# WangFeng18/3d-gaussian-splatting

Measured on NVIDIA H100. Metric: render+backward FPS @1080p (2.4M Gaussians), higher is better.
Workload: dtype f32

## Files before the change

### 3d-gaussian-splatting_b200/csrc/blend.cu

```cuda
#include <cstdlib>
#include <type_traits>

#include "internal.h"

namespace {

constexpr int FWD_THREADS = 64;
constexpr int FWD_PX = 4;
constexpr int FWD_STAGES = 2;

template <int FWD_CH>
struct FwdSmem {
  float4 A[FWD_STAGES][FWD_CH];
  float4 C[FWD_STAGES][FWD_CH];
  float2 B[FWD_STAGES][FWD_CH + 2];
  uint64_t full[FWD_STAGES];
};

template <typename SM, int CH>
__device__ __forceinline__ void issue_chunk(SM& sm, int stage, const float4* __restrict__ pA,
                                            const float2* __restrict__ pB, const float4* __restrict__ pC,
                                            int base, int n, int shift) {
  uint32_t bytes_a = (uint32_t)n * 16u;
  uint32_t nb = (uint32_t)(n + shift + 1) & ~1u;
// ... 26 lines not shown
    return make_float2(t.x, t.y);
  }
  __device__ __forceinline__ float4 c(int j) const {
    const float4 t = R[j * recw + 1];
    return make_float4(t.z, t.w, R[j * recw + 2].x, 0.f);
  }
  __device__ __forceinline__ float depth(int j) const { return R[j * recw + 2].y; }
  __device__ __forceinline__ uint32_t slot(int j, int tx, int ty) const {
    const float4 cc = R[j * recw + 2];
    const uint32_t rxy = __float_as_uint(cc.z), rwh = __float_as_uint(cc.w);
    const uint32_t off = __float_as_uint(R[j * recw + 3].x);
    return off + ((uint32_t)ty - (rxy >> 16)) * (rwh & 0xffffu) + ((uint32_t)tx - (rxy & 0xffffu));
  }
};

template <int CH, int STAGES, int RECW>
struct GatherRing {
  float4 rec[STAGES][CH * RECW];
  uint64_t full[STAGES];
};

template <int NT, int CH>
struct GatherIds {
  uint32_t id[(CH + NT - 1) / NT];
  __device__ __forceinline__ void load(const uint32_t* __restrict__ ids, int base, int n, int tid) {
#pragma unroll
    for (int u = 0; u < (CH + NT - 1) / NT; ++u) {
      const int i = tid + u * NT;
      id[u] = i < n ? __ldg(ids + base + i) : 0u;
    }
  }
};

template <typename SM, int NT, int CH, int RECW>
__device__ __forceinline__ void gather_issue(SM& sm, int stage, const GsRec* __restrict__ grec,
                                             const uint32_t* __restrict__ goff, const GatherIds<NT, CH>& g, int n,
                                             int tid) {
#pragma unroll
  for (int u = 0; u < (CH + NT - 1) / NT; ++u) {
    const int i = tid + u * NT;
    if (i < n) {
      const float4* src = reinterpret_cast<const float4*>(grec + g.id[u]);
      const uint32_t dst = gs_smem_u32(&sm.rec[stage][i * RECW]);
#pragma unroll
      for (int q = 0; q < 3; ++q)
        asm volatile("cp.async.cg.shared.global [%0], [%1], 16;" ::"r"(dst + 16u * q), "l"(src + q) : "memory");
      if (RECW == 4)
        asm volatile("cp.async.ca.shared.global [%0], [%1], 4;" ::"r"(dst + 48u), "l"(goff + g.id[u]) : "memory");
    }
  }
  asm volatile("cp.async.mbarrier.arrive.noinc.shared::cta.b64 [%0];" ::"r"(gs_smem_u32(&sm.full[stage])) : "memory");
}

template <int FWD_CH, int PX, bool GATHER, bool AUX = false, bool BATCH = false>
__device__ __forceinline__ void blend_fwd_body(const float4* __restrict__ pA, const float2* __restrict__ pB,
                                               const float4* __restrict__ pC, const GsRec* __restrict__ grec,
                                               const uint32_t* __restrict__ ids, const int* __restrict__ tile_accum,
                                               int wp, int hp, int ntx, float fx, float fy, float* __restrict__ image,
                                               int* __restrict__ tile_neff, float* __restrict__ final_img, GsCrop crop,
                                               GsAuxOut aux, const GsView* __restrict__ views) {
  static_assert(!AUX || GATHER, "the aux outputs read |p_c| from the gathered records");
  static_assert(!BATCH || GATHER, "batched frames run the gather path");
  using Smem = typename std::conditional<GATHER, GatherRing<FWD_CH, FWD_STAGES, 3>, FwdSmem<FWD_CH>>::type;
  __shared__ __align__(16) Smem sm;
  const int tile = blockIdx.x;
  const int tid = threadIdx.x;
  const int tx = tile % ntx, ty = tile / ntx;
  int lty = ty;
  if constexpr (BATCH) {
    const int v = ty / (hp / GS_TILE);
    lty = ty - v * (hp / GS_TILE);
    fx = views[v].fx;
    fy = views[v].fy;
    if (final_img) final_img += (size_t)v * crop.width * crop.height * 3;
    if (aux.aux_final) aux.aux_final += (size_t)v * crop.width * crop.height * 2;
  }
  constexpr int FWD_PX = PX, TPR = GS_TILE / PX, NTHREADS = 256 / PX;
  const int ix0 = tx * GS_TILE + (tid % TPR) * FWD_PX;
  const int iy = ty * GS_TILE + (tid / TPR);
  const int iyv = lty * GS_TILE + (tid / TPR);
  float px[FWD_PX];
#pragma unroll
  for (int p = 0; p < FWD_PX; ++p) px[p] = gs_pixel_coord(ix0 + p, wp, fx);
  const float py = gs_pixel_coord(iyv, hp, fy);

  const int start = tile_accum[tile];
  const int cnt = tile_accum[tile + 1] - start;
  const int shift = start & 1;
  const int nchunks = (cnt + FWD_CH - 1) / FWD_CH;

  if (tid == 0) {
    for (int s = 0; s < FWD_STAGES; ++s) gs_mbar_init(&sm.full[s], GATHER ? NTHREADS : 1);
    gs_fence_barrier_init();
  }
  __syncthreads();
  GatherIds<NTHREADS, FWD_CH> gid;
  if constexpr (GATHER) {
    for (int k = 0; k < FWD_STAGES && k < nchunks; ++k) {
      gid.load(ids, start + k * FWD_CH, min(FWD_CH, cnt - k * FWD_CH), tid);
      gather_issue<Smem, NTHREADS, FWD_CH, 3>(sm, k, grec, nullptr, gid, min(FWD_CH, cnt - k * FWD_CH), tid);
    }
    if (FWD_STAGES < nchunks) gid.load(ids, start + FWD_STAGES * FWD_CH, min(FWD_CH, cnt - FWD_STAGES * FWD_CH), tid);
  } else if (tid == 0) {
    for (int k = 0; k < FWD_STAGES && k < nchunks; ++k)
      issue_chunk<Smem, FWD_CH>(sm, k, pA, pB, pC, start + k * FWD_CH, min(FWD_CH, cnt - k * FWD_CH), shift);
  }

  float T[FWD_PX], cr[FWD_PX], cg[FWD_PX], cb[FWD_PX], dep[FWD_PX];
#pragma unroll
  for (int p = 0; p < FWD_PX; ++p) {
    T[p] = 1.f;
    cr[p] = cg[p] = cb[p] = 0.f;
    dep[p] = 0.f;
  }
  int consumed = cnt;
  int k = 0;
  for (; k < nchunks; ++k) {
    const int stage = k % FWD_STAGES;
    gs_mbar_wait(&sm.full[stage], (uint32_t)((k / FWD_STAGES) & 1));
    const int n = min(FWD_CH, cnt - k * FWD_CH);
    StageView<GATHER> sv;
    if constexpr (GATHER) {
      sv.R = sm.rec[stage];
      sv.recw = 3;
    } else {
      sv.A = sm.A[stage];
      sv.C = sm.C[stage];
      sv.B = sm.B[stage] + shift;
    }

#define GS_FWD_BODY(J)                                                                      \
  {                                                                                         \
    const float4 a = sv.a(J);                                                               \
    const float2 b = sv.b(J);                                                               \
    const float4 c = sv.c(J);                                                               \
    const float dy = py - a.y;                                                              \
    const float m1 = a.w * dy;                                                              \
    const float ev = fmaf(-b.x * dy, dy, b.y);                                              \
    float t = 0.f;                                                                          \
    if constexpr (AUX) t = sv.depth(J);                                                     \
    _Pragma("unroll") for (int p = 0; p < FWD_PX; ++p) {                                    \
      const float dx = px[p] - a.x;                                                         \
      const float eu = fmaf(a.z, dx, -m1);                                                  \
      const float alpha = gs_ex2(fmaf(-dx, eu, ev));  \
      const float w = (T[p] > GS_T_STOP) ? alpha * T[p] : 0.f;                              \
      cr[p] = fmaf(c.x, w, cr[p]);                                                          \
      cg[p] = fmaf(c.y, w, cg[p]);                                                          \
      cb[p] = fmaf(c.z, w, cb[p]);                                                          \
      if constexpr (AUX) dep[p] = fmaf(t, w, dep[p]);                                       \
      T[p] -= w;                                                                            \
    }                                                                                       \
  }
    int j = 0;
    bool warp_dead = false;
    for (; j + 4 <= n; j += 4) {
#pragma unroll
      for (int u = 0; u < 4; ++u) GS_FWD_BODY(j + u)
      bool dead = true;
#pragma unroll
      for (int p = 0; p < FWD_PX; ++p) dead = dead && !(T[p] > GS_T_STOP);
      if (__all_sync(0xffffffffu, dead)) {
        warp_dead = true;
        break;
      }
    }
    if (!warp_dead)
      for (; j < n; ++j) GS_FWD_BODY(j)
#undef GS_FWD_BODY

    bool dead = true;
#pragma unroll
    for (int p = 0; p < FWD_PX; ++p) dead = dead && !(T[p] > GS_T_STOP);
    const int all_dead = NTHREADS == 32 ? __all_sync(0xffffffffu, dead) : __syncthreads_and(dead);
    if (NTHREADS == 32) __syncwarp();
    if (all_dead) {
      consumed = min(cnt, (k + 1) * FWD_CH);
      break;
    }
    if (k + FWD_STAGES < nchunks) {
      const int kn = k + FWD_STAGES;
      if constexpr (GATHER) {
        gather_issue<Smem, NTHREADS, FWD_CH, 3>(sm, stage, grec, nullptr, gid, min(FWD_CH, cnt - kn * FWD_CH), tid);
        if (kn + 1 < nchunks) gid.load(ids, start + (kn + 1) * FWD_CH, min(FWD_CH, cnt - (kn + 1) * FWD_CH), tid);
      } else if (tid == 0)
        issue_chunk<Smem, FWD_CH>(sm, stage, pA, pB, pC, start + kn * FWD_CH, min(FWD_CH, cnt - kn * FWD_CH), shift);
    }
  }
  if (tid == 0 && k < nchunks) {
    for (int kk = k + 1; kk < nchunks && kk < k + FWD_STAGES; ++kk)
      gs_mbar_wait(&sm.full[kk % FWD_STAGES], (uint32_t)((kk / FWD_STAGES) & 1));
  }
  if constexpr (AUX) {
#pragma unroll
    for (int p = 0; p < FWD_PX; ++p) {
      cr[p] = fmaf(T[p], aux.bg[0], cr[p]);
      cg[p] = fmaf(T[p], aux.bg[1], cg[p]);
      cb[p] = fmaf(T[p], aux.bg[2], cb[p]);
    }
    float ab[FWD_PX * 2];
#pragma unroll
    for (int p = 0; p < FWD_PX; ++p) {
      ab[2 * p] = dep[p];
      ab[2 * p + 1] = 1.f - T[p];
    }
    if (aux.aux) {
      float4* o = reinterpret_cast<float4*>(aux.aux + ((size_t)iy * wp + ix0) * 2);
#pragma unroll
      for (int q = 0; q < FWD_PX / 2; ++q) o[q] = make_float4(ab[4 * q], ab[4 * q + 1], ab[4 * q + 2], ab[4 * q + 3]);
    }
    if (aux.aux_final) {
#pragma unroll
      for (int p = 0; p < FWD_PX; ++p) {
        const int x = ix0 + p - crop.left, y = iyv - crop.top;
        if (x >= 0 && x < crop.width && y >= 0 && y < crop.height)
          *reinterpret_cast<float2*>(aux.aux_final + ((size_t)y * crop.width + x) * 2) = make_float2(ab[2 * p], ab[2 * p + 1]);
      }
    }
  }
  {
    float ob[FWD_PX * 3];
#pragma unroll
    for (int p = 0; p < FWD_PX; ++p) {
      ob[3 * p] = cr[p];
      ob[3 * p + 1] = cg[p];
      ob[3 * p + 2] = cb[p];
    }
    float4* o = reinterpret_cast<float4*>(image + ((size_t)iy * wp + ix0) * 3);
#pragma unroll
    for (int q = 0; q < FWD_PX * 3 / 4; ++q) o[q] = make_float4(ob[4 * q], ob[4 * q + 1], ob[4 * q + 2], ob[4 * q + 3]);
  }
  if (final_img) {
#pragma unroll
    for (int p = 0; p < FWD_PX; ++p)
      gs_store_final(final_img, ix0 + p, iyv, crop.left, crop.top, crop.width, crop.height, cr[p], cg[p], cb[p]);
  }
  if (tile_neff && tid == 0) tile_neff[tile] = consumed;
}

template <int FWD_CH, int PX, bool GATHER, bool AUX = false>
__global__ void __launch_bounds__(256 / PX) blend_fwd_kernel(const float4* __restrict__ pA,
                                                                 const float2* __restrict__ pB,
                                                                 const float4* __restrict__ pC,
                                                                 const GsRec* __restrict__ grec,
                                                                 const uint32_t* __restrict__ ids,
                                                                 const int* __restrict__ tile_accum, int wp, int hp,
                                                                 int ntx, float fx, float fy,
                                                                 float* __restrict__ image,
                                                                 int* __restrict__ tile_neff,
                                                                 float* __restrict__ final_img, GsCrop crop,
                                                                 GsAuxOut aux) {
  blend_fwd_body<FWD_CH, PX, GATHER, AUX>(pA, pB, pC, grec, ids, tile_accum, wp, hp, ntx, fx, fy, image, tile_neff,
                                          final_img, crop, aux, nullptr);
}

template <bool AUX>
__global__ void __launch_bounds__(64) blend_fwd_batch_kernel(const GsRec* __restrict__ grec,
                                                             const uint32_t* __restrict__ ids,
                                                             const int* __restrict__ tile_accum, int wp, int hp,
                                                             int ntx, const GsView* __restrict__ views,
                                                             float* __restrict__ image, int* __restrict__ tile_neff,
                                                             float* __restrict__ final_img, GsCrop crop, GsAuxOut aux) {
  blend_fwd_body<128, 4, true, AUX, true>(nullptr, nullptr, nullptr, grec, ids, tile_accum, wp, hp, ntx, 0.f, 0.f,
                                          image, tile_neff, final_img, crop, aux, views);
}

constexpr int BWD_STAGES = 2;
constexpr int BWD_NV = 9;

template <int WARPS, int BWD_CH>
struct BwdSmem {
  float4 A[BWD_STAGES][BWD_CH];
  float4 C[BWD_STAGES][BWD_CH];
  float2 B[BWD_STAGES][BWD_CH + 2];
  uint64_t full[BWD_STAGES];
  float partial[WARPS][BWD_CH * BWD_NV];
};

template <int WARPS, int BWD_CH>
__global__ void __launch_bounds__(32 * WARPS) blend_bwd_kernel(const float4* __restrict__ pA,
                                                                const float2* __restrict__ pB,
                                                                const float4* __restrict__ pC,
                                                                const int* __restrict__ tile_accum, int wp, int hp,
                                                                int ntx, float fx, float fy,
                                                                const float* __restrict__ image,
                                                                const float* __restrict__ grad_image,
                                                                float* __restrict__ grad_inst, int grad_is_final,
                                                                GsCrop crop, uint32_t* __restrict__ row_epoch,
                                                                uint32_t epoch, int* __restrict__ tile_neff_b) {
  constexpr int THREADS = 32 * WARPS;
  constexpr int PX = 256 / THREADS;
  constexpr int TPR = GS_TILE / PX;
  using Smem = BwdSmem<WARPS, BWD_CH>;
  __shared__ __align__(16) Smem sm;
  const int tile = blockIdx.x;
  const int tid = threadIdx.x, warp = tid >> 5, lane = tid & 31;
  const int tx = tile % ntx, ty = tile / ntx;
  const int start = tile_accum[tile];
  const int cnt = tile_accum[tile + 1] - start;
  if (cnt == 0) return;
  const int shift = start & 1;
  const int nchunks = (cnt + BWD_CH - 1) / BWD_CH;

  const int ix0 = tx * GS_TILE + (tid % TPR) * PX;
  const int iy = ty * GS_TILE + (tid / TPR);
  float px[PX];
#pragma unroll
  for (int p = 0; p < PX; ++p) px[p] = gs_pixel_coord(ix0 + p, wp, fx);
  const float py = gs_pixel_coord(iy, hp, fy);

  float T[PX], R[PX], gr[PX], gg[PX], gb[PX];
  {
    const size_t off = ((size_t)iy * wp + ix0) * 3;
    const float4* im = reinterpret_cast<const float4*>(image + off);
    float gbuf[PX * 3], ibuf[PX * 3];
#pragma unroll
    for (int q = 0; q < PX * 3 / 4; ++q) {
// ... 958 lines not shown
                                                                      float* __restrict__ g_cov) {
  int i = blockIdx.x * 256 + threadIdx.x;
  if (i >= m) return;
  const float* row = grad_inst + (size_t)i * gw;
  float4 cv = reinterpret_cast<const float4*>(cov)[i];
  float det = cv.x * cv.w - cv.y * cv.z;
  double pn = 2.0 * (double)det + 1e-14;
  float sc = (float)((double)GS_LOG2E / pn);
  float kk = 2.f * sc * sc / GS_LOG2E;
  float d_ca = row[2], d_cb = row[3], d_cc = row[4];
  float gsc = d_ca * cv.w + d_cb * (cv.y + cv.z) + d_cc * cv.x;
  g_pos[3 * i] = row[0];
  g_pos[3 * i + 1] = row[1];
  reinterpret_cast<float4*>(g_cov)[i] = make_float4(d_cc * sc - gsc * kk * cv.w, d_cb * sc + gsc * kk * cv.z,
                                                    d_cb * sc + gsc * kk * cv.y, d_ca * sc - gsc * kk * cv.x);
  g_opa[i] = opa[i] > 0.f ? row[5] / (opa[i] * GS_LN2) : 0.f;
  for (int q = 0; q < d; ++q) g_rgb[(size_t)i * d + q] = row[6 + q];
}

struct LegacyWs {
  float4* pA;
  float2* pB;
  float4* pC;
  float* grad_inst;
};

inline size_t align_up(size_t x, size_t a) { return (x + a - 1) / a * a; }

inline size_t legacy_ws_layout(int m, int d, LegacyWs* ws, char* base) {
  size_t off = 0;
  size_t mm = (size_t)(m > 0 ? m : 0);
  size_t crow = d == 3 ? 16 : (size_t)gs_sh_stream_width(d) * 4;
  size_t grow = d == 3 ? (size_t)GS_GREC * 4 : (size_t)gs_sh_grad_width(d) * 4;
  if (ws) ws->pA = reinterpret_cast<float4*>(base + off);
  off += align_up(mm * 16, 256);
  if (ws) ws->pC = reinterpret_cast<float4*>(base + off);
  off += align_up(mm * crow + 16, 256);
  if (ws) ws->pB = reinterpret_cast<float2*>(base + off);
  off += align_up((mm + 2) * 8, 256);
  if (ws) ws->grad_inst = reinterpret_cast<float*>(base + off);
  off += align_up(mm * grow, 256);
  return off;
}

}

cudaError_t gs_launch_blend_fwd(const float4* pA, const float2* pB, const float4* pC, const GsRec* grec,
                                const uint32_t* ids, const int* tile_accum, const GsFrameGeom& g, float* image,
                                int* tile_neff, float* final_img, const GsCrop& crop, cudaStream_t st,
                                const GsAuxOut* aux) {
  const GsTuning& tn = gs_tuning();
  const bool gather = grec != nullptr;
  if (aux) {
    blend_fwd_kernel<128, 4, true, true><<<g.n_tiles, 64, 0, st>>>(pA, pB, pC, grec, ids, tile_accum, g.wp, g.hp, g.ntx,
                                                                  g.fx, g.fy, image, tile_neff, final_img, crop, *aux);
    return cudaGetLastError();
  }
  if (!gather && tn.fwd_kernel != 0) {
    blend_fwd_ws_kernel<<<g.n_tiles, WSF_CONS + 32, 0, st>>>(pA, pB, pC, tile_accum, g.wp, g.hp, g.ntx, g.fx, g.fy, image,
                                                             tile_neff, final_img, crop);
    return cudaGetLastError();
  }
  const int ch = tn.fwd_ch;
#define GS_FWD_LAUNCH(CH, PX, GA)                                                                                   \
  blend_fwd_kernel<CH, PX, GA><<<g.n_tiles, 256 / PX, 0, st>>>(pA, pB, pC, grec, ids, tile_accum, g.wp, g.hp, g.ntx, \
                                                               g.fx, g.fy, image, tile_neff, final_img, crop, GsAuxOut{})
#define GS_FWD_CH(PX, GA)                     \
  if (ch == 64) GS_FWD_LAUNCH(64, PX, GA);    \
  else if (ch == 256) GS_FWD_LAUNCH(256, PX, GA); \
  else GS_FWD_LAUNCH(128, PX, GA)
  if (gather) {
    if (tn.fwd_px == 8) { GS_FWD_CH(8, true); } else { GS_FWD_CH(4, true); }
  } else {
    if (tn.fwd_px == 8) { GS_FWD_CH(8, false); } else { GS_FWD_CH(4, false); }
  }
#undef GS_FWD_CH
#undef GS_FWD_LAUNCH
  return cudaGetLastError();
}

cudaError_t gs_launch_blend_bwd(const float4* pA, const float2* pB, const float4* pC, const GsRec* grec,
                                const uint32_t* ids, const uint32_t* goff, const int* tile_accum, const GsFrameGeom& g,
                                const float* image,
                                const float* grad_image, float* grad_inst, int grad_is_final, const GsCrop& crop,
                                uint32_t* row_epoch, uint32_t epoch, int* tile_neff_b, cudaStream_t st,
                                const float* aux, const float* grad_aux, bool absgrad) {
  const GsTuning& tn = gs_tuning();
  const bool gather = grec != nullptr;
  if (gather && !row_epoch) return cudaErrorInvalidValue;
  if (absgrad) {
    if (!gather || (grad_aux && !aux)) return cudaErrorInvalidValue;
#define GS_BWD2_ABS(AX, RP)                                                                                        \
  blend_bwd2_kernel<8, false, 4, 3, 10, 4, true, 32, AX, RP, true><<<g.n_tiles, 32, 0, st>>>(                       \
      pA, pB, pC, grec, ids, goff, tile_accum, g.wp, g.hp, g.ntx, g.fx, g.fy, image, grad_image, grad_inst,         \
      grad_is_final, crop, row_epoch, epoch, tile_neff_b, aux, grad_aux)
    if (grad_aux && tn.blend_repack) GS_BWD2_ABS(true, true);
    else if (grad_aux) GS_BWD2_ABS(true, false);
    else if (tn.blend_repack) GS_BWD2_ABS(false, true);
    else GS_BWD2_ABS(false, false);
#undef GS_BWD2_ABS
    return cudaGetLastError();
  }
  if (grad_aux) {
    if (!gather || !aux) return cudaErrorInvalidValue;
#define GS_BWD2_AUX(RP)                                                                                            \
  blend_bwd2_kernel<8, false, 4, 3, 10, 4, true, 32, true, RP><<<g.n_tiles, 32, 0, st>>>(                           \
      pA, pB, pC, grec, ids, goff, tile_accum, g.wp, g.hp, g.ntx, g.fx, g.fy, image, grad_image, grad_inst,         \
      grad_is_final, crop, row_epoch, epoch, tile_neff_b, aux, grad_aux)
    if (tn.blend_repack) GS_BWD2_AUX(true);
    else GS_BWD2_AUX(false);
#undef GS_BWD2_AUX
    return cudaGetLastError();
  }
  if (tn.bwd_kernel != 0 || gather) {
#define GS_BWD2C(PX, WS, UNR, ST, MINB, RQ, GA, CH)                                                                 \
  blend_bwd2_kernel<PX, WS, UNR, ST, MINB, RQ, GA, CH><<<g.n_tiles, 256 / PX + (WS ? 32 : 0), 0, st>>>(              \
      pA, pB, pC, grec, ids, goff, tile_accum, g.wp, g.hp, g.ntx, g.fx, g.fy, image, grad_image, grad_inst,          \
      grad_is_final,                                                                                                 \
      crop, row_epoch, epoch, tile_neff_b, nullptr, nullptr)
#define GS_BWD2(PX, WS, UNR, ST, MINB, RQ, GA) GS_BWD2C(PX, WS, UNR, ST, MINB, RQ, GA, 64)
    const int key = ((((tn.bwd_px * 10 + tn.bwd_ws) * 10 + tn.bwd_unroll) * 10 + tn.bwd_stages) * 10 + tn.bwd_rq) * 100 +
                    tn.bwd_minb;
    if (gather && tn.bwd_ch == 32) {
#define GS_BWD2_SHIPPED()                                                                                          \
  if (tn.blend_repack)                                                                                             \
// ... 72 lines not shown

static bool shipped_rgb_bwd_knobs(const GsTuning& tn) {
  return tn.bwd_kernel != 0 && tn.bwd_px == 8 && tn.bwd_ws == 0 && tn.bwd_unroll == 4 && tn.bwd_stages == 3 &&
         tn.bwd_rq == 4 && tn.bwd_minb == 10 && tn.bwd_ch == 32;
}

int gs_blend_aux_supported(int d, bool forward, bool backward) {
  const GsTuning& tn = gs_tuning();
  if (!tn.gather)
    return gs_set_error_msg(GS_ERR_UNSUPPORTED, "depth / alpha / background: the packed path (gs_tune(\"gather\", 0)) has no aux kernel");
  if (d != 3) {
    if (backward && (gs_sh_tc_mode(d) & 6) == 6)
      return gs_set_error_msg(GS_ERR_UNSUPPORTED,
                              "depth / alpha gradients: the two-pixel tensor-core SH backward (sh_tc bit 2) has no aux kernel");
    return 0;
  }
  if (forward && (tn.fwd_kernel != 0 || tn.fwd_ch != 128 || tn.fwd_px != 4))
    return gs_set_error_msg(GS_ERR_UNSUPPORTED,
                            "depth / alpha / background: only the shipped forward blend knobs (fwd_kernel 0, fwd_ch 128, fwd_px 4) have an aux kernel");
  if (backward && !shipped_rgb_bwd_knobs(tn))
    return gs_set_error_msg(GS_ERR_UNSUPPORTED,
                            "depth / alpha gradients: only the shipped backward blend knobs have an aux kernel");
  return 0;
}

int gs_blend_absgrad_supported(int d, bool gather) {
  const GsTuning& tn = gs_tuning();
  if (d != 3)
    return gs_set_error_msg(GS_ERR_UNSUPPORTED,
                            "densify statistics: absgrad needs the RGB blend (RGB or per-Gaussian SH colour); SH colour "
                            "evaluated per pixel has only grad2d");
  if (!gather)
    return gs_set_error_msg(GS_ERR_UNSUPPORTED,
                            "densify statistics: absgrad is not available on the packed path (gs_tune(\"gather\", 0))");
  if (!shipped_rgb_bwd_knobs(tn))
    return gs_set_error_msg(GS_ERR_UNSUPPORTED,
                            "densify statistics: absgrad needs the shipped backward blend knobs");
  return 0;
}

int gs_blend_batch_supported() {
  const GsTuning& tn = gs_tuning();
  if (!tn.gather)
    return gs_set_error_msg(GS_ERR_UNSUPPORTED, "batched frame: the packed path (gs_tune(\"gather\", 0)) has no batched kernel");
  if (tn.fwd_kernel != 0 || tn.fwd_ch != 128 || tn.fwd_px != 4 || !shipped_rgb_bwd_knobs(tn) || !tn.blend_repack)
    return gs_set_error_msg(GS_ERR_UNSUPPORTED,
                            "batched frame: only the shipped RGB blend knobs (with the live-pixel repack) have batched kernels");
  return 0;
}

cudaError_t gs_launch_blend_fwd_batch(const GsRec* grec, const uint32_t* ids, const int* tile_accum,
                                      const GsFrameGeom& g, const GsView* views, float* image, int* tile_neff,
                                      float* final_img, const GsCrop& crop, cudaStream_t st, const GsAuxOut* aux) {
  if (aux)
    blend_fwd_batch_kernel<true><<<g.n_tiles, 64, 0, st>>>(grec, ids, tile_accum, g.wp, g.hp, g.ntx, views, image,
                                                           tile_neff, final_img, crop, *aux);
  else
    blend_fwd_batch_kernel<false><<<g.n_tiles, 64, 0, st>>>(grec, ids, tile_accum, g.wp, g.hp, g.ntx, views, image,
                                                            tile_neff, final_img, crop, GsAuxOut{});
  return cudaGetLastError();
}

cudaError_t gs_launch_blend_bwd_batch(const GsRec* grec, const uint32_t* ids, const uint32_t* goff,
                                      const int* tile_accum, const GsFrameGeom& g, const GsView* views,
                                      const float* image, const float* grad_image, float* grad_inst, int grad_is_final,
                                      const GsCrop& crop, uint32_t* row_epoch, uint32_t epoch, int* tile_neff_b,
                                      cudaStream_t st, const float* aux, const float* grad_aux, bool absgrad) {
  if (!row_epoch || (grad_aux && !aux)) return cudaErrorInvalidValue;
#define GS_BWD2_BATCH(AX, AB)                                                                                      \
  blend_bwd2_batch_kernel<AX, AB><<<g.n_tiles, 32, 0, st>>>(nullptr, nullptr, nullptr, grec, ids, goff, tile_accum, \
                                                            g.wp, g.hp, g.ntx, 0.f, 0.f, image, grad_image,         \
                                                            grad_inst, grad_is_final, crop, row_epoch, epoch,       \
                                                            tile_neff_b, aux, grad_aux, views)
  if (grad_aux && absgrad) GS_BWD2_BATCH(true, true);
  else if (grad_aux) GS_BWD2_BATCH(true, false);
  else if (absgrad) GS_BWD2_BATCH(false, true);
  else GS_BWD2_BATCH(false, false);
#undef GS_BWD2_BATCH
  return cudaGetLastError();
}

extern "C" size_t gs_draw_workspace_bytes(int m, int d) {
  if (d != 3 && gs_sh_basis_count(d) == 0) return 0;
  return legacy_ws_layout(m, d, nullptr, nullptr);
}

static int check_draw_args(const char* fn, int m, int d, int wp, int hp, int weight_normalize, int sigmoid,
                           size_t ws_bytes, void* ws) {
  if (m < 0 || wp <= 0 || hp <= 0 || (wp % GS_TILE) || (hp % GS_TILE))
    return gs_set_error_msg(GS_ERR_INVALID_ARG, fn);
  if (weight_normalize || sigmoid || (d != 3 && gs_sh_basis_count(d) == 0)) return gs_set_error_msg(GS_ERR_UNSUPPORTED, fn);
  if (m > 0 && (ws == nullptr || ws_bytes < gs_draw_workspace_bytes(m, d)))
    return gs_set_error_msg(GS_ERR_INVALID_ARG, fn);
  return 0;
}

extern "C" int gs_draw_fwd(const float* pos, const float* rgb, const float* opa, const float* cov,
                           const int* tile_n_point_accum, int m, int d, int width_padded, int height_padded,
                           float focal_x, float focal_y, int weight_normalize, int sigmoid, const float* rays_o,
                           const float* lefttop, const float* vec_dx, const float* vec_dy, float* image,
                           void* workspace, size_t workspace_bytes, gs_stream_t stream) {
  int rc = check_draw_args("gs_draw_fwd: bad/unsupported arguments", m, d, width_padded, height_padded,
                           weight_normalize, sigmoid, workspace_bytes, workspace);
  if (rc) return rc;
  if (d != 3 && (!rays_o || !lefttop || !vec_dx || !vec_dy))
    return gs_set_error_msg(GS_ERR_INVALID_ARG, "gs_draw_fwd: SH colour needs rays_o / lefttop / vec_dx / vec_dy");
  cudaStream_t st = (cudaStream_t)stream;
  LegacyWs ws{};
  legacy_ws_layout(m, d, &ws, static_cast<char*>(workspace));
  if (m > 0) {
    if (d == 3)
      legacy_pack_kernel<<<(m + 255) / 256, 256, 0, st>>>(pos, rgb, opa, cov, m, ws.pA, ws.pB, ws.pC);
// ... 77 lines not shown
```

### 3d-gaussian-splatting_b200/csrc/internal.h

```cpp
#pragma once
#include <cuda_runtime.h>
#include <stdint.h>

#include "../../include/gs_b200.h"
#include "project.cuh"

#define GS_GREC 12

struct GsFrameGeom {
  int width, height, wp, hp, ntx, nty, n_tiles;
  float fx, fy;
};

struct GsCrop {
  int left, top, width, height;
};

struct GsAuxOut {
  float bg[3];
  float* aux;
  float* aux_final;
};

#ifdef __CUDACC__
__device__ __forceinline__ void gs_store_aux(const GsAuxOut& ax, int ix, int iy, int wp, const GsCrop& crop,
                                             float depth, float alpha) {
  if (ax.aux) *reinterpret_cast<float2*>(ax.aux + ((size_t)iy * wp + ix) * 2) = make_float2(depth, alpha);
  const int x = ix - crop.left, y = iy - crop.top;
  if (ax.aux_final && x >= 0 && x < crop.width && y >= 0 && y < crop.height)
    *reinterpret_cast<float2*>(ax.aux_final + ((size_t)y * crop.width + x) * 2) = make_float2(depth, alpha);
}
template <int PX>
__device__ __forceinline__ void gs_load_aux_grad(const float* __restrict__ aux, const float* __restrict__ grad_aux,
                                                 int grad_is_final, int ix0, int iy, int wp, const GsCrop& crop,
                                                 float (&gD)[PX], float (&gA)[PX], float (&R)[PX]) {
#pragma unroll
  for (int p = 0; p < PX; ++p) {
    const size_t off = ((size_t)iy * wp + ix0 + p) * 2;
    const float2 da = *reinterpret_cast<const float2*>(aux + off);
    float2 g = make_float2(0.f, 0.f);
    if (!grad_is_final) {
      g = *reinterpret_cast<const float2*>(grad_aux + off);
    } else {
      const int x = ix0 + p - crop.left, y = iy - crop.top;
      if (x >= 0 && x < crop.width && y >= 0 && y < crop.height)
        g = *reinterpret_cast<const float2*>(grad_aux + ((size_t)y * crop.width + x) * 2);
    }
    gD[p] = g.x;
    gA[p] = g.y;
    R[p] = fmaf(g.x, da.x, fmaf(g.y, da.y, R[p]));
  }
}
#endif

struct GsRayPtrs {
  const float *rays_o, *lefttop, *dx, *dy;
};

struct GsTuning {
  int fwd_kernel;
  int fwd_ch;
  int bwd_kernel;
  int bwd_px;
  int bwd_ws;
  int bwd_unroll;
  int bwd_stages;
  int bwd_minb;
  int bwd_rq;
  int fwd_px;
  int bwd_ch;
  int strict;
  int gather;
  int sh_tc;
  int blend_repack;
};
GsTuning& gs_tuning();

void gs_count_launch(int n = 1);

int gs_sh_basis_count(int d);
int gs_sh_stream_width(int d);
int gs_sh_grad_width(int d);
int gs_sh_tc_mode(int d);
cudaError_t gs_launch_blend_sh_fwd(const float4* pA, const float2* pB, const float* pS, const GsRec* grec,
                                   const float* rgb, const uint32_t* ids, const uint32_t* goff , int d,
                                   const int* tile_accum,
                                   const GsFrameGeom& g, const GsRayPtrs& r, float* image, int* tile_neff,
                                   float* final_img, const GsCrop& crop, cudaStream_t st,
                                   const GsAuxOut* aux = nullptr );
cudaError_t gs_launch_blend_sh_bwd(const float4* pA, const float2* pB, const float* pS, const GsRec* grec,
                                   const float* rgb, const uint32_t* ids, const uint32_t* goff , int d,
                                   const int* tile_accum,
                                   const GsFrameGeom& g, const GsRayPtrs& r, const float* image,
                                   const float* grad_image, float* grad_inst, int grad_is_final, const GsCrop& crop,
                                   uint32_t* row_epoch, uint32_t epoch, int* tile_neff_b, cudaStream_t st,
                                   const float* aux = nullptr, const float* grad_aux = nullptr );

cudaError_t gs_launch_blend_sh_fwd_tc(const GsRec* grec, const float* rgb, const uint32_t* ids, int d,
                                      const int* tile_accum, const GsFrameGeom& g, const GsRayPtrs& r, float* image,
                                      int* tile_neff, float* final_img, const GsCrop& crop, cudaStream_t st,
                                      const GsAuxOut* aux = nullptr);
cudaError_t gs_launch_blend_sh_bwd_tc(const GsRec* grec, const float* rgb, const uint32_t* ids, const uint32_t* goff, int d,
                                      const int* tile_accum, const GsFrameGeom& g, const GsRayPtrs& r, const float* image,
                                      const float* grad_image, float* grad_inst, int grad_is_final, const GsCrop& crop,
                                      uint32_t* row_epoch, uint32_t epoch, int* tile_neff_b, cudaStream_t st,
                                      const float* aux = nullptr, const float* grad_aux = nullptr);

cudaError_t gs_launch_fused_project(const float* pos, const float* rgb, const float* opa, const float* quat,
                                    const float* scale, int n, int d, int scale_act, const GsCam& cam,
                                    const GsTileGrid& grid, float near_plane, float half_w, float half_h,
                                    GsRec* rec, uint2* rect ,
                                    uint32_t* count, uint32_t* dkey, int64_t* mask, unsigned int* n_visible, cudaStream_t st,
                                    bool sh_gaussian = false ,
                                    const GsFilter2d* filt = nullptr );

struct GsView {
  GsCam cam;
  GsTileGrid grid;
  GsFilter2d filt;
  float half_w, half_h, fx, fy;
};

cudaError_t gs_launch_fused_project_batch(const float* pos, const float* rgb, const float* opa, const float* quat,
                                          const float* scale, int n, int n_views, int d, int scale_act,
                                          const GsView* views, float near_plane, GsRec* rec ,
                                          uint2* rect , uint32_t* count , uint32_t* dkey ,
                                          int64_t* mask , unsigned int* n_visible,
// ... 116 lines not shown
```

### 3d-gaussian-splatting_b200/csrc/render.cu

```cuda
#include <cub/device/device_radix_sort.cuh>
#include <cub/device/device_scan.cuh>
#include <cub/iterator/counting_input_iterator.cuh>
#include <cub/iterator/transform_input_iterator.cuh>

#include <cmath>
#include <cstdio>
#include <cstdlib>
#include <cstring>
#include <new>

#include "internal.h"

struct GsCountInSortedOrder {
  const uint32_t* count;
  const uint32_t* perm;
  uint32_t n;
  __host__ __device__ __forceinline__ uint32_t operator()(uint32_t i) const { return i < n ? count[perm[i]] : 0u; }
};

static thread_local char g_err[512] = {0};

int gs_set_error(cudaError_t e, const char* what) {
  snprintf(g_err, sizeof(g_err), "CUDA error %d (%s) at %s", (int)e, cudaGetErrorString(e), what);
  return (int)e;
}
int gs_set_error_msg(int code, const char* what) {
  snprintf(g_err, sizeof(g_err), "%s", what);
  return code;
}
extern "C" const char* gs_last_error(void) { return g_err; }
extern "C" int gs_abi_version(void) { return 2; }

static int tune_env(const char* name, int dflt) {
  const char* e = getenv(name);
  return e ? atoi(e) : dflt;
}
GsTuning& gs_tuning() {
  static GsTuning t = {tune_env("GS_TUNE_FWD_KERNEL", 0),  tune_env("GS_TUNE_FWD_CH", 128),   tune_env("GS_TUNE_BWD_KERNEL", 1),
                       tune_env("GS_TUNE_BWD_PX", 8),      tune_env("GS_TUNE_BWD_WS", 0),     tune_env("GS_TUNE_BWD_UNROLL", 4),
                       tune_env("GS_TUNE_BWD_STAGES", 3),  tune_env("GS_TUNE_BWD_MINB", 10),  tune_env("GS_TUNE_BWD_RQ", 4),
                       tune_env("GS_TUNE_FWD_PX", 4),      tune_env("GS_TUNE_BWD_CH", 32),    tune_env("GS_TUNE_STRICT", 0),
                       tune_env("GS_TUNE_GATHER", 1),      tune_env("GS_TUNE_SH_TC", -1),     tune_env("GS_TUNE_BLEND_REPACK", 1)};
  return t;
}
extern "C" int gs_tune(const char* name, int value) {
  if (!name) return gs_set_error_msg(GS_ERR_INVALID_ARG, "gs_tune: null name");
  GsTuning& t = gs_tuning();
  struct { const char* k; int* v; } tab[] = {{"fwd_kernel", &t.fwd_kernel}, {"fwd_ch", &t.fwd_ch},
                                             {"bwd_kernel", &t.bwd_kernel}, {"bwd_px", &t.bwd_px},
                                             {"bwd_ws", &t.bwd_ws},         {"bwd_unroll", &t.bwd_unroll},
                                             {"bwd_stages", &t.bwd_stages}, {"bwd_minb", &t.bwd_minb},
                                             {"bwd_rq", &t.bwd_rq},         {"fwd_px", &t.fwd_px},
                                             {"gather", &t.gather},         {"bwd_ch", &t.bwd_ch},
                                             {"strict", &t.strict},         {"sh_tc", &t.sh_tc},
                                             {"blend_repack", &t.blend_repack}};
  for (auto& e : tab)
    if (!strcmp(e.k, name)) {
      *e.v = value;
      return 0;
    }
  return gs_set_error_msg(GS_ERR_INVALID_ARG, "gs_tune: unknown knob");
}

#include <atomic>
static std::atomic<unsigned long long> g_launches{0};
void gs_count_launch(int n) { g_launches.fetch_add((unsigned long long)n, std::memory_order_relaxed); }
extern "C" unsigned long long gs_kernel_launches(void) { return g_launches.load(std::memory_order_relaxed); }

struct GsAllocator {
  gs_alloc_fn alloc = nullptr;
  gs_free_fn free = nullptr;
  void* user = nullptr;
};
static thread_local const GsAllocator* g_cur_alloc = nullptr;

struct DevBuf {
  void* p = nullptr;
  size_t cap = 0;
  const GsAllocator* owner = nullptr;
  void drop(cudaStream_t st, bool sync) {
    if (!p) return;
    if (owner && owner->free) {
      owner->free(p, owner->user);
    } else {
      if (sync) cudaStreamSynchronize(st);
      cudaFree(p);
    }
    p = nullptr;
    cap = 0;
  }
  cudaError_t reserve(size_t bytes, cudaStream_t st) {
    if (bytes <= cap) return cudaSuccess;
    drop(st, true);
    size_t want = bytes + bytes / 8 + 256;
    const GsAllocator* a = g_cur_alloc;
    if (a && a->alloc) {
      p = a->alloc(want, a->user, (gs_stream_t)st);
      if (!p) return cudaErrorMemoryAllocation;
      owner = a;
    } else {
      cudaError_t e = cudaMalloc(&p, want);
      if (e != cudaSuccess) return e;
      owner = nullptr;
    }
    cap = want;
    return cudaSuccess;
  }
  void release() { drop(nullptr, false); }
// ... 1004 lines not shown
```

Measured before the change: 488.7.

## Repack live pixels across warp lanes in forward blend as pixels saturate

Adds a forward-blend repacking step. At segment and chunk boundaries, each warp counts the pixels that are still unsaturated. When enough have terminated, it retires the finished pixels by writing them to the image, then redistributes the survivors so each lane holds 2 or 1 pixels via warp shuffles. This targets wasted alpha-blend work on lanes whose pixels have already hit the transmittance cutoff. The cost is shuffle-heavy bookkeeping, more code paths specialised on pixel count, and scattered pixel stores. It is enabled by default through a new tuning knob.

```diff
diff --git a/3d-gaussian-splatting_b200/csrc/blend.cu b/3d-gaussian-splatting_b200/csrc/blend.cu
--- a/3d-gaussian-splatting_b200/csrc/blend.cu
+++ b/3d-gaussian-splatting_b200/csrc/blend.cu
@@ -102,7 +102,113 @@
   asm volatile("cp.async.mbarrier.arrive.noinc.shared::cta.b64 [%0];" ::"r"(gs_smem_u32(&sm.full[stage])) : "memory");
 }
 
-template <int FWD_CH, int PX, bool GATHER, bool AUX = false, bool BATCH = false>
+constexpr int FWD_RP = 32;
+
+template <bool AUX, typename Retire>
+__device__ __forceinline__ void fwd_repack(int warp, int lane, int& S, int& row, uint32_t& cols, int& npx,
+                                           float (&px)[4], float& py, float (&T)[4], float (&cr)[4], float (&cg)[4],
+                                           float (&cb)[4], float (&dep)[4], Retire&& retire) {
+  uint32_t mask = 0;
+#pragma unroll
+  for (int p = 0; p < 4; ++p) mask |= T[p] > GS_T_STOP ? 1u << p : 0u;
+  const int c = __popc(mask);
+  if (__reduce_add_sync(0xffffffffu, c) > 16 * S) return;
+  const int wr = row - 8 * warp;
+  int live = 0;
+#pragma unroll
+  for (int r = 0; r < 8; ++r) {
+    const int v = __reduce_add_sync(0xffffffffu, wr == r ? c : 0);
+    if (lane == r) live = v;
+  }
+  int ns = S;
+  while (ns > 1 && __reduce_add_sync(0xffffffffu, (live + ns / 2 - 1) / (ns / 2)) <= 32) ns /= 2;
+  if (ns == S) return;
+
+#pragma unroll
+  for (int p = 0; p < 4; ++p)
+    if (p < npx && !((mask >> p) & 1u)) retire((int)((cols >> (4 * p)) & 15u), row, T[p], cr[p], cg[p], cb[p], dep[p]);
+  int excl = c;
+#pragma unroll
+  for (int o = 1; o < 32; o <<= 1) {
+    const int t = __shfl_up_sync(0xffffffffu, excl, o);
+    if (lane >= o) excl += t;
+  }
+  excl -= c;
+  int sc = (((live + ns - 1) / ns) << 16) | live;
+  const int own = sc;
+#pragma unroll
+  for (int o = 1; o < 8; o <<= 1) {
+    const int t = __shfl_up_sync(0xffffffffu, sc, o);
+    if (lane >= o) sc += t;
+  }
+  sc -= own;
+  int nr = GS_TILE, src = 0, n = 0;
+#pragma unroll
+  for (int r = 0; r < 8; ++r) {
+    const int s = __shfl_sync(0xffffffffu, sc, r), lr = __shfl_sync(0xffffffffu, live, r);
+    const int q = lane - (s >> 16);
+    if (q >= 0 && q * ns < lr) {
+      nr = 8 * warp + r;
+      src = (s & 0xffff) + q * ns;
+      n = min(ns, lr - q * ns);
+    }
+  }
+  int sl[2], sp[2];
+  uint32_t ncols = 0;
+#pragma unroll
+  for (int q = 0; q < 2; ++q) {
+    const int e = src + q;
+    int l = 0;
+#pragma unroll
+    for (int b = 16; b > 0; b >>= 1) {
+      const int t = __shfl_sync(0xffffffffu, excl, (l + b) & 31);
+      if (l + b < 32 && t <= e) l += b;
+    }
+    const int k = e - __shfl_sync(0xffffffffu, excl, l);
+    const uint32_t m = __shfl_sync(0xffffffffu, mask, l);
+    const uint32_t cl = __shfl_sync(0xffffffffu, cols, l);
+    int pos = 0, cnt = 0;
+#pragma unroll
+    for (int p = 0; p < 4; ++p)
+      if ((m >> p) & 1u) {
+        if (cnt == k) pos = p;
+        ++cnt;
+      }
+    sl[q] = l;
+    sp[q] = pos;
+    if (q < n) ncols |= ((cl >> (4 * pos)) & 15u) << (4 * q);
+  }
+  const float npy = __shfl_sync(0xffffffffu, py, sl[0]);
+  auto move = [&](float (&v)[4]) {
+    float nv[2];
+#pragma unroll
+    for (int q = 0; q < 2; ++q) {
+      float acc = 0.f;
+#pragma unroll
+      for (int p = 0; p < 4; ++p) {
+        const float t = __shfl_sync(0xffffffffu, v[p], sl[q]);
+        if (sp[q] == p) acc = t;
+      }
+      nv[q] = q < n ? acc : 0.f;
+    }
+    v[0] = nv[0];
+    v[1] = nv[1];
+    v[2] = v[3] = 0.f;
+  };
+  move(px);
+  move(T);
+  move(cr);
+  move(cg);
+  move(cb);
+  if constexpr (AUX) move(dep);
+  if (n) py = npy;
+  row = nr;
+  cols = ncols;
+  npx = n;
+  S = ns;
+}
+
+template <int FWD_CH, int PX, bool GATHER, bool AUX = false, bool BATCH = false, bool REPACK = false>
 __device__ __forceinline__ void blend_fwd_body(const float4* __restrict__ pA, const float2* __restrict__ pB,
                                                const float4* __restrict__ pC, const GsRec* __restrict__ grec,
                                                const uint32_t* __restrict__ ids, const int* __restrict__ tile_accum,
@@ -111,6 +217,7 @@
                                                GsAuxOut aux, const GsView* __restrict__ views) {
   static_assert(!AUX || GATHER, "the aux outputs read |p_c| from the gathered records");
   static_assert(!BATCH || GATHER, "batched frames run the gather path");
+  static_assert(!REPACK || (GATHER && PX == 4 && FWD_CH % FWD_RP == 0), "the repack deals 4-pixel lanes at segment ends");
   using Smem = typename std::conditional<GATHER, GatherRing<FWD_CH, FWD_STAGES, 3>, FwdSmem<FWD_CH>>::type;
   __shared__ __align__(16) Smem sm;
   const int tile = blockIdx.x;
@@ -132,7 +239,10 @@
   float px[FWD_PX];
 #pragma unroll
   for (int p = 0; p < FWD_PX; ++p) px[p] = gs_pixel_coord(ix0 + p, wp, fx);
-  const float py = gs_pixel_coord(iyv, hp, fy);
+  float py = gs_pixel_coord(iyv, hp, fy);
+  int S = FWD_PX, row = tid / TPR, npx = FWD_PX;
+  uint32_t cols = 0;
+  if constexpr (REPACK) cols = ((uint32_t)(tid % TPR) * 4u) * 0x1111u + 0x3210u;
 
   const int start = tile_accum[tile];
   const int cnt = tile_accum[tile + 1] - start;
@@ -163,6 +273,24 @@
     cr[p] = cg[p] = cb[p] = 0.f;
     dep[p] = 0.f;
   }
+  auto store_px = [&](int col, int r, float t, float pr, float pg, float pb, float d) {
+    const int ix = tx * GS_TILE + col, iyp = ty * GS_TILE + r, iyq = lty * GS_TILE + r;
+    if constexpr (AUX) {
+      pr = fmaf(t, aux.bg[0], pr);
+      pg = fmaf(t, aux.bg[1], pg);
+      pb = fmaf(t, aux.bg[2], pb);
+      const float2 da = make_float2(d, 1.f - t);
+      if (aux.aux) *reinterpret_cast<float2*>(aux.aux + ((size_t)iyp * wp + ix) * 2) = da;
+      const int x = ix - crop.left, y = iyq - crop.top;
+      if (aux.aux_final && x >= 0 && x < crop.width && y >= 0 && y < crop.height)
+        *reinterpret_cast<float2*>(aux.aux_final + ((size_t)y * crop.width + x) * 2) = da;
+    }
+    float* o = image + ((size_t)iyp * wp + ix) * 3;
+    o[0] = pr;
+    o[1] = pg;
+    o[2] = pb;
+    if (final_img) gs_store_final(final_img, ix, iyq, crop.left, crop.top, crop.width, crop.height, pr, pg, pb);
+  };
   int consumed = cnt;
   int k = 0;
   for (; k < nchunks; ++k) {
@@ -179,6 +307,8 @@
       sv.B = sm.B[stage] + shift;
     }
 
+    auto run = [&](auto np, int j, const int jend) -> int {
+      constexpr int NP = decltype(np)::value;
 #define GS_FWD_BODY(J)                                                                      \
   {                                                                                         \
     const float4 a = sv.a(J);                                                               \
@@ -189,7 +319,7 @@
     const float ev = fmaf(-b.x * dy, dy, b.y);                                              \
     float t = 0.f;                                                                          \
     if constexpr (AUX) t = sv.depth(J);                                                     \
-    _Pragma("unroll") for (int p = 0; p < FWD_PX; ++p) {                                    \
+    _Pragma("unroll") for (int p = 0; p < NP; ++p) {                                        \
       const float dx = px[p] - a.x;                                                         \
       const float eu = fmaf(a.z, dx, -m1);                                                  \
       const float alpha = gs_ex2(fmaf(-dx, eu, ev));  \
@@ -201,22 +331,36 @@
       T[p] -= w;                                                                            \
     }                                                                                       \
   }
-    int j = 0;
-    bool warp_dead = false;
-    for (; j + 4 <= n; j += 4) {
-#pragma unroll
-      for (int u = 0; u < 4; ++u) GS_FWD_BODY(j + u)
-      bool dead = true;
-#pragma unroll
-      for (int p = 0; p < FWD_PX; ++p) dead = dead && !(T[p] > GS_T_STOP);
-      if (__all_sync(0xffffffffu, dead)) {
-        warp_dead = true;
-        break;
-      }
-    }
-    if (!warp_dead)
-      for (; j < n; ++j) GS_FWD_BODY(j)
+      bool warp_dead = false;
+      for (; j + 4 <= jend; j += 4) {
+#pragma unroll
+        for (int u = 0; u < 4; ++u) GS_FWD_BODY(j + u)
+        bool dead = true;
+#pragma unroll
+        for (int p = 0; p < NP; ++p) dead = dead && !(T[p] > GS_T_STOP);
+        if (__all_sync(0xffffffffu, dead)) {
+          warp_dead = true;
+          break;
+        }
+      }
+      if (!warp_dead)
+        for (; j < jend; ++j) GS_FWD_BODY(j)
 #undef GS_FWD_BODY
+      return warp_dead ? n : j;
+    };
+    if constexpr (REPACK) {
+      for (int j = 0; j < n;) {
+        const int jend = min(n, j + FWD_RP);
+        switch (S) {
+          case 4: j = run(std::integral_constant<int, 4>{}, j, jend); break;
+          case 2: j = run(std::integral_constant<int, 2>{}, j, jend); break;
+          default: j = run(std::integral_constant<int, 1>{}, j, jend); break;
+        }
+        if (j < n && S > 1) fwd_repack<AUX>(tid >> 5, tid & 31, S, row, cols, npx, px, py, T, cr, cg, cb, dep, store_px);
+      }
+    } else {
+      run(std::integral_constant<int, FWD_PX>{}, 0, n);
+    }
 
     bool dead = true;
 #pragma unroll
@@ -235,10 +379,22 @@
       } else if (tid == 0)
         issue_chunk<Smem, FWD_CH>(sm, stage, pA, pB, pC, start + kn * FWD_CH, min(FWD_CH, cnt - kn * FWD_CH), shift);
     }
+    if constexpr (REPACK)
+      if (S > 1 && k + 1 < nchunks)
+        fwd_repack<AUX>(tid >> 5, tid & 31, S, row, cols, npx, px, py, T, cr, cg, cb, dep, store_px);
   }
   if (tid == 0 && k < nchunks) {
     for (int kk = k + 1; kk < nchunks && kk < k + FWD_STAGES; ++kk)
       gs_mbar_wait(&sm.full[kk % FWD_STAGES], (uint32_t)((kk / FWD_STAGES) & 1));
+  }
+  if constexpr (REPACK) {
+    if (S < FWD_PX) {
+#pragma unroll
+      for (int p = 0; p < FWD_PX; ++p)
+        if (p < npx) store_px((int)((cols >> (4 * p)) & 15u), row, T[p], cr[p], cg[p], cb[p], dep[p]);
+      if (tile_neff && tid == 0) tile_neff[tile] = consumed;
+      return;
+    }
   }
   if constexpr (AUX) {
 #pragma unroll
@@ -287,7 +443,7 @@
   if (tile_neff && tid == 0) tile_neff[tile] = consumed;
 }
 
-template <int FWD_CH, int PX, bool GATHER, bool AUX = false>
+template <int FWD_CH, int PX, bool GATHER, bool AUX = false, bool REPACK = false>
 __global__ void __launch_bounds__(256 / PX) blend_fwd_kernel(const float4* __restrict__ pA,
                                                                  const float2* __restrict__ pB,
                                                                  const float4* __restrict__ pC,
@@ -299,19 +455,19 @@
                                                                  int* __restrict__ tile_neff,
                                                                  float* __restrict__ final_img, GsCrop crop,
                                                                  GsAuxOut aux) {
-  blend_fwd_body<FWD_CH, PX, GATHER, AUX>(pA, pB, pC, grec, ids, tile_accum, wp, hp, ntx, fx, fy, image, tile_neff,
-                                          final_img, crop, aux, nullptr);
-}
-
-template <bool AUX>
+  blend_fwd_body<FWD_CH, PX, GATHER, AUX, false, REPACK>(pA, pB, pC, grec, ids, tile_accum, wp, hp, ntx, fx, fy, image,
+                                                         tile_neff, final_img, crop, aux, nullptr);
+}
+
+template <bool AUX, bool REPACK>
 __global__ void __launch_bounds__(64) blend_fwd_batch_kernel(const GsRec* __restrict__ grec,
                                                              const uint32_t* __restrict__ ids,
                                                              const int* __restrict__ tile_accum, int wp, int hp,
                                                              int ntx, const GsView* __restrict__ views,
                                                              float* __restrict__ image, int* __restrict__ tile_neff,
                                                              float* __restrict__ final_img, GsCrop crop, GsAuxOut aux) {
-  blend_fwd_body<128, 4, true, AUX, true>(nullptr, nullptr, nullptr, grec, ids, tile_accum, wp, hp, ntx, 0.f, 0.f,
-                                          image, tile_neff, final_img, crop, aux, views);
+  blend_fwd_body<128, 4, true, AUX, true, REPACK>(nullptr, nullptr, nullptr, grec, ids, tile_accum, wp, hp, ntx, 0.f,
+                                                  0.f, image, tile_neff, final_img, crop, aux, views);
 }
 
 constexpr int BWD_STAGES = 2;
@@ -1376,8 +1532,13 @@
   const GsTuning& tn = gs_tuning();
   const bool gather = grec != nullptr;
   if (aux) {
-    blend_fwd_kernel<128, 4, true, true><<<g.n_tiles, 64, 0, st>>>(pA, pB, pC, grec, ids, tile_accum, g.wp, g.hp, g.ntx,
-                                                                  g.fx, g.fy, image, tile_neff, final_img, crop, *aux);
+    if (tn.blend_fwd_repack)
+      blend_fwd_kernel<128, 4, true, true, true><<<g.n_tiles, 64, 0, st>>>(pA, pB, pC, grec, ids, tile_accum, g.wp, g.hp,
+                                                                          g.ntx, g.fx, g.fy, image, tile_neff, final_img,
+                                                                          crop, *aux);
+    else
+      blend_fwd_kernel<128, 4, true, true><<<g.n_tiles, 64, 0, st>>>(pA, pB, pC, grec, ids, tile_accum, g.wp, g.hp, g.ntx,
+                                                                    g.fx, g.fy, image, tile_neff, final_img, crop, *aux);
     return cudaGetLastError();
   }
   if (!gather && tn.fwd_kernel != 0) {
@@ -1394,7 +1555,12 @@
   else if (ch == 256) GS_FWD_LAUNCH(256, PX, GA); \
   else GS_FWD_LAUNCH(128, PX, GA)
   if (gather) {
-    if (tn.fwd_px == 8) { GS_FWD_CH(8, true); } else { GS_FWD_CH(4, true); }
+    if (tn.fwd_px == 8) { GS_FWD_CH(8, true); }
+    else if (ch == 128 && tn.blend_fwd_repack)
+      blend_fwd_kernel<128, 4, true, false, true><<<g.n_tiles, 64, 0, st>>>(pA, pB, pC, grec, ids, tile_accum, g.wp, g.hp,
+                                                                           g.ntx, g.fx, g.fy, image, tile_neff, final_img,
+                                                                           crop, GsAuxOut{});
+    else { GS_FWD_CH(4, true); }
   } else {
     if (tn.fwd_px == 8) { GS_FWD_CH(8, false); } else { GS_FWD_CH(4, false); }
   }
@@ -1573,12 +1739,15 @@
 cudaError_t gs_launch_blend_fwd_batch(const GsRec* grec, const uint32_t* ids, const int* tile_accum,
                                       const GsFrameGeom& g, const GsView* views, float* image, int* tile_neff,
                                       float* final_img, const GsCrop& crop, cudaStream_t st, const GsAuxOut* aux) {
-  if (aux)
-    blend_fwd_batch_kernel<true><<<g.n_tiles, 64, 0, st>>>(grec, ids, tile_accum, g.wp, g.hp, g.ntx, views, image,
-                                                           tile_neff, final_img, crop, *aux);
-  else
-    blend_fwd_batch_kernel<false><<<g.n_tiles, 64, 0, st>>>(grec, ids, tile_accum, g.wp, g.hp, g.ntx, views, image,
-                                                            tile_neff, final_img, crop, GsAuxOut{});
+#define GS_FWD_BATCH(AX, RP, AUXV)                                                                                   \
+  blend_fwd_batch_kernel<AX, RP><<<g.n_tiles, 64, 0, st>>>(grec, ids, tile_accum, g.wp, g.hp, g.ntx, views, image,     \
+                                                           tile_neff, final_img, crop, AUXV)
+  const bool rp = gs_tuning().blend_fwd_repack != 0;
+  if (aux && rp) GS_FWD_BATCH(true, true, *aux);
+  else if (aux) GS_FWD_BATCH(true, false, *aux);
+  else if (rp) GS_FWD_BATCH(false, true, GsAuxOut{});
+  else GS_FWD_BATCH(false, false, GsAuxOut{});
+#undef GS_FWD_BATCH
   return cudaGetLastError();
 }
 
diff --git a/3d-gaussian-splatting_b200/csrc/internal.h b/3d-gaussian-splatting_b200/csrc/internal.h
--- a/3d-gaussian-splatting_b200/csrc/internal.h
+++ b/3d-gaussian-splatting_b200/csrc/internal.h
@@ -73,6 +73,7 @@
   int gather;
   int sh_tc;
   int blend_repack;
+  int blend_fwd_repack;
 };
 GsTuning& gs_tuning();
 
diff --git a/3d-gaussian-splatting_b200/csrc/render.cu b/3d-gaussian-splatting_b200/csrc/render.cu
--- a/3d-gaussian-splatting_b200/csrc/render.cu
+++ b/3d-gaussian-splatting_b200/csrc/render.cu
@@ -40,7 +40,8 @@
                        tune_env("GS_TUNE_BWD_PX", 8),      tune_env("GS_TUNE_BWD_WS", 0),     tune_env("GS_TUNE_BWD_UNROLL", 4),
                        tune_env("GS_TUNE_BWD_STAGES", 3),  tune_env("GS_TUNE_BWD_MINB", 10),  tune_env("GS_TUNE_BWD_RQ", 4),
                        tune_env("GS_TUNE_FWD_PX", 4),      tune_env("GS_TUNE_BWD_CH", 32),    tune_env("GS_TUNE_STRICT", 0),
-                       tune_env("GS_TUNE_GATHER", 1),      tune_env("GS_TUNE_SH_TC", -1),     tune_env("GS_TUNE_BLEND_REPACK", 1)};
+                       tune_env("GS_TUNE_GATHER", 1),      tune_env("GS_TUNE_SH_TC", -1),     tune_env("GS_TUNE_BLEND_REPACK", 1),
+                       tune_env("GS_TUNE_BLEND_FWD_REPACK", 1)};
   return t;
 }
 extern "C" int gs_tune(const char* name, int value) {
@@ -53,7 +54,7 @@
                                              {"bwd_rq", &t.bwd_rq},         {"fwd_px", &t.fwd_px},
                                              {"gather", &t.gather},         {"bwd_ch", &t.bwd_ch},
                                              {"strict", &t.strict},         {"sh_tc", &t.sh_tc},
-                                             {"blend_repack", &t.blend_repack}};
+                                             {"blend_repack", &t.blend_repack}, {"blend_fwd_repack", &t.blend_fwd_repack}};
   for (auto& e : tab)
     if (!strcmp(e.k, name)) {
       *e.v = value;
```

New measurement: 494.8, median of 6. No clear change (+1.3%).
